# UltimateSoftware/surge

Measured on AMD Instinct MI355X. Metric: events/sec replayed, higher is better.
Workload: dtype int32/int64 adds + bit-copied f64

## Files before the change

### surge_amd/csrc/engine.hip

```cpp
#include <algorithm>
#include <atomic>
#include <cstdio>
#include <cstdlib>
#include <cstring>
#include <mutex>
#include <new>
#include <shared_mutex>
#include <string>
#include <vector>

#include "replay_internal.h"
#include "f64_text.h"
#include "state_parse.h"

using namespace surge;

namespace {

thread_local std::string g_last_error;

struct DevBuf {
  void* ptr = nullptr;
  size_t cap = 0;
  hipError_t reserve(size_t bytes) {
// ... 50 lines not shown
  std::mutex err_mu;

  DevBuf own_seg_off, own_events, own_init, own_state;
  const int64_t* d_seg_off = nullptr;
  const uint4* d_events = nullptr;
  const uint4* d_init = nullptr;
  uint4* d_state = nullptr;
  int64_t n_agg = 0, n_events = 0;
  bool bound = false;
  bool log_valid = false;

  CsrAnalysis an{};
  DevBuf d_analysis, nz_off, nz_map, block_counts;
  int64_t n_nz = 0;
  DevBuf perm, counter;
  DevBuf ix_arena, ix_cnt;
  bool perm_valid = false;
  struct ChunkIndex {
    DevBuf arena;
    void *v_start = nullptr, *v_len = nullptr, *v_info = nullptr, *v_seg = nullptr, *v_side = nullptr, *r_slot0 = nullptr, *r_c = nullptr, *r_out = nullptr;
    int64_t n_vrows = 0, n_cut_rows = 0;
    uint32_t T = 0;
    void release() {
      arena.release();
      v_start = v_len = v_info = v_seg = v_side = r_slot0 = r_c = r_out = nullptr;
      n_vrows = n_cut_rows = 0;
      T = 0;
    }
  };
  ChunkIndex cidx;
// ... 275 lines not shown
  if (extra) *extra = base + o_extra;
  return SURGE_OK;
}

void index_scratch_release(surge_replay_handle* h) {
  h->ix_arena.release();
  h->ix_cnt.release();
}

int32_t run_slots(surge_replay_handle* h, FoldParams& p, const int64_t* off, int64_t n_seg, bool cache_perm) {
  if (!cache_perm || !h->perm_valid) {
    HIPCHK(h, h->perm.reserve((size_t)(n_seg > 0 ? n_seg : 1) * 8));
    IndexScratch sc;
    const int32_t rcs = index_scratch(h, n_seg, false, cache_perm ? h->an.max_len : -1, 0, &sc);
    if (rcs != SURGE_OK) return rcs;
    HIPCHK(h, launch_sort_by_length(off, n_seg, sc, (int64_t*)h->perm.ptr, h->stream));
    h->perm_valid = cache_perm;
  }
  p.seg_off = off;
  p.plan = (const int64_t*)h->perm.ptr;
  {
    const int32_t rcd = dispenser_begin(h, p);
    if (rcd != SURGE_OK) return rcd;
  }
  p.n_seg = n_seg;
  const int64_t groups = (n_seg + kWave - 1) / kWave;
  const int le = env_lane_events("SURGE_REPLAY_LE_SLOTS", h->spec ? 16 : 8) == 16 ? 16 : 8;
  int64_t per_cu = le == 8 ? (h->spec ? 12 : 14) : 8;
  if (const char* v = std::getenv("SURGE_REPLAY_SLOTS_WAVES")) per_cu = std::atoi(v) > 0 ? std::atoi(v) : per_cu;
  const int64_t slots = (int64_t)h->n_cus * per_cu;
  const int64_t n_waves = groups < slots ? groups : slots;
  hipEvent_t e0, e1;
// ... 155 lines not shown
  if (!h) return SURGE_OK;
  DeviceGuard g(h->device);
  (void)hipStreamSynchronize(h->stream);
  if (h->comm) comm_destroy(h->comm);
  h->comm = nullptr;
  for (int k = 0; k < 2; ++k) {
    if (h->pinned[k]) (void)hipHostFree(h->pinned[k]);
    h->pinned[k] = nullptr;
    if (h->ev_staged[k]) (void)hipEventDestroy(h->ev_staged[k]);
    h->ev_staged[k] = nullptr;
  }
  if (h->host_flags) (void)hipHostFree(h->host_flags);
  h->host_flags = nullptr;
  h->cidx.release();
  h->tidx.release();
  DevBuf* bufs[] = {&h->gb_temp, &h->gb_u32, &h->gb_flags, &h->gb_agg_idx, &h->gb_events, &h->published, &h->gathered[0], &h->gathered[1], &h->f64_tables, &h->nan_count, &h->sd_ptab, &h->sd_counts, &h->sd_last, &h->sd_status, &h->ix_arena, &h->ix_cnt, &h->stage_keys, &h->stage_events, &h->t_tiles, &h->t_gsub, &h->perm, &h->counter, &h->own_seg_off, &h->own_events, &h->own_init, &h->own_state, &h->d_analysis, &h->nz_off,
                    &h->nz_map, &h->block_counts, &h->plan, &h->batch_group_agg, &h->batch_group_off,
                    &h->batch_events, &h->poison_count, &h->gather_idx, &h->gather_out, &h->scan_totals};
  for (DevBuf* b : bufs) b->release();
  hipEvent_t evs[] = {h->ev_total0, h->ev_total1, h->ev_h0, h->ev_h1, h->ev_i0, h->ev_i1, h->ev_r0, h->ev_r1};
  for (hipEvent_t ev : evs)
    if (ev) (void)hipEventDestroy(ev);
  for (auto& pr : h->fold_events) {
    (void)hipEventDestroy(pr.first);
    (void)hipEventDestroy(pr.second);
  }
  delete h;
  return SURGE_OK;
}

const char* surge_replay_last_error(const surge_replay_handle* h) {
// ... 29 lines not shown
}

int32_t surge_replay_bind_device_csr(surge_replay_handle* h, const int64_t* d_seg_off, int64_t n_agg,
                                     const void* d_events, int64_t n_events, const void* d_init_state,
                                     void* d_state_out) {
  if (!h) return fail(nullptr, SURGE_E_INVALID, "handle is NULL");
  if (n_agg < 0 || n_events < 0) return fail(h, SURGE_E_INVALID, "negative size");
  if (!d_seg_off) return fail(h, SURGE_E_INVALID, "seg_off is NULL");
  if (n_events > 0 && !d_events) return fail(h, SURGE_E_INVALID, "events is NULL");
  if (((uintptr_t)d_events & 15) || ((uintptr_t)d_init_state & 15) || ((uintptr_t)d_state_out & 15) ||
      ((uintptr_t)d_seg_off & 7))
    return fail(h, SURGE_E_INVALID, "device buffers must be 16-byte aligned (seg_off: 8)");
  DeviceGuard g(h->device);
  h->bound = false;
  h->perm_valid = false;
  h->cidx.T = 0;
  h->tidx.T = 0;
  h->tiled_valid = false;
  h->index_timed = h->relayout_timed = false;
  h->index_algo = 0;
  h->d_seg_off = d_seg_off;
  h->d_events = (const uint4*)d_events;
  h->d_init = (const uint4*)d_init_state;
  h->n_agg = n_agg;
  h->n_events = n_events;
  if (d_state_out) {
    h->d_state = (uint4*)d_state_out;
  } else {
    HIPCHK(h, h->own_state.reserve((size_t)n_agg * 64));
    h->d_state = (uint4*)h->own_state.ptr;
// ... 141 lines not shown
                               (int64_t*)ci.v_start, (uint32_t*)ci.v_len, (uint32_t*)ci.v_info, (int64_t*)ci.v_seg,
                               (int64_t*)ci.r_slot0, (uint32_t*)ci.r_c, (int64_t*)ci.r_out, h->stream));
  ci.T = T;
  return SURGE_OK;
}

int32_t ensure_index(surge_replay_handle* h, const FoldPlan& pl) {
  if (h->n_agg <= 0 || pl.span <= 0) return SURGE_OK;
  const int64_t* off = h->an.n_empty > 0 ? (const int64_t*)h->nz_off.ptr : h->d_seg_off;
  const int64_t n_seg = h->an.n_empty > 0 ? h->n_nz : h->n_agg;
  if (pl.use == SURGE_ALGO_SORTED && !h->perm_valid) {
    HIPCHK(h, h->perm.reserve((size_t)n_seg * 8));
    IndexScratch sc;
    const int32_t rcs = index_scratch(h, n_seg, false, h->an.max_len, 0, &sc);
    if (rcs != SURGE_OK) return rcs;
    HIPCHK(h, hipEventRecord(h->ev_i0, h->stream));
    HIPCHK(h, launch_sort_by_length(off, n_seg, sc, (int64_t*)h->perm.ptr, h->stream));
    HIPCHK(h, hipEventRecord(h->ev_i1, h->stream));
    h->perm_valid = true;
    h->index_timed = true;
    h->relayout_timed = false;
    h->index_algo = SURGE_ALGO_SORTED;
  } else if (pl.use == SURGE_ALGO_CHUNKED && h->cidx.T != pl.chunk_T) {
    HIPCHK(h, hipEventRecord(h->ev_i0, h->stream));
    const int32_t rc = build_chunk_index(h, h->cidx, off, n_seg, pl.chunk_T, true);
    if (rc != SURGE_OK) return rc;
    HIPCHK(h, hipEventRecord(h->ev_i1, h->stream));
    h->index_timed = true;
    h->relayout_timed = false;
    h->index_algo = SURGE_ALGO_CHUNKED;
  } else if (pl.use == SURGE_ALGO_TILED && (!h->tiled_valid || h->tidx.T != pl.chunk_T)) {
    h->tiled_valid = false;
    HIPCHK(h, hipEventRecord(h->ev_i0, h->stream));
    const int32_t rc = build_chunk_index(h, h->tidx, off, n_seg, pl.chunk_T, false);
// ... 275 lines not shown
      p.n_seg = h->n_agg;
      hipEvent_t e0, e1;
      const int32_t rc = next_fold_events(h, &e0, &e1);
      if (rc != SURGE_OK) return rc;
      HIPCHK(h, hipEventRecord(e0, h->stream));
      HIPCHK(h, launch_fold_short(p, h->stream));
      HIPCHK(h, hipEventRecord(e1, h->stream));
      h->st.n_tasks = (int32_t)((h->n_agg + 63) / 64);
    } else if (use == SURGE_ALGO_SORTED) {
      const int le = env_lane_events("SURGE_REPLAY_LE_SORTED", 16);
      const int64_t* off = h->an.n_empty > 0 ? (const int64_t*)h->nz_off.ptr : h->d_seg_off;
      const int64_t n_seg = h->an.n_empty > 0 ? h->n_nz : h->n_agg;
      if (h->an.n_empty > 0) p.out_map = (const int64_t*)h->nz_map.ptr;
      p.seg_off = off;
      p.plan = (const int64_t*)h->perm.ptr;
      {
        const int32_t rcd = dispenser_begin(h, p);
        if (rcd != SURGE_OK) return rcd;
      }
      p.n_seg = n_seg;
      const int64_t groups = (n_seg + kWave - 1) / kWave;
      int64_t per_cu = le == 8 ? 12 : (le == 16 ? 8 : 4);
      if (const char* v = std::getenv("SURGE_REPLAY_SORTED_WAVES")) per_cu = std::atoi(v) > 0 ? std::atoi(v) : per_cu;
      const int64_t slots = (int64_t)h->n_cus * per_cu;
      const int64_t n_waves = groups < slots ? groups : slots;
      hipEvent_t e0, e1;
      const int32_t rc = next_fold_events(h, &e0, &e1);
      if (rc != SURGE_OK) return rc;
      const V1Kernels* lanes = lane_spec(h, p);
      HIPCHK(h, hipEventRecord(e0, h->stream));
// ... 82 lines not shown
  if (n_groups == 0 || n_events == 0) return SURGE_OK;
  if (!d_group_agg || !d_group_off || !d_events) return fail(h, SURGE_E_INVALID, "NULL batch buffer");
  if ((uintptr_t)d_events & 15) return fail(h, SURGE_E_INVALID, "events must be 16-byte aligned");
  DeviceGuard g(h->device);
  FoldParams p;
  fill_params(h, p);
  p.events = (const uint4*)d_events;
  p.n_events = n_events;
  p.init = h->d_state;
  p.out = h->d_state;
  p.out_map = d_group_agg;
  HIPCHK(h, hipEventRecord(h->ev_total0, h->stream));
  if (h->v2) std::memset(p.table, 0, sizeof(p.table));
  const int32_t rc = h->v2 ? run_slots(h, p, d_group_off, n_groups, false) : run_flat(h, p, d_group_off, n_groups, n_events);
  if (rc != SURGE_OK) return rc;
  if (h->v2) h->perm_valid = false;
  HIPCHK(h, hipEventRecord(h->ev_total1, h->stream));
  h->timing_valid = true;
  h->st.last_algo = h->v2 ? SURGE_ALGO_SLOTS : SURGE_ALGO_FLAT;
  h->st.n_folds += 1;
  h->st.n_poisoned = -1;
  h->fold_epoch.fetch_add(1);
  return SURGE_OK;
}

int32_t surge_replay_append_fold(surge_replay_handle* h, const int64_t* group_agg, const int64_t* group_off,
                                 int64_t n_groups, const void* events, int64_t n_events) {
  if (!h) return fail(nullptr, SURGE_E_INVALID, "handle is NULL");
  if (!h->bound) return fail(h, SURGE_E_STATE, "append_fold before load_csr/bind_device_csr");
  if (n_groups < 0 || n_events < 0) return fail(h, SURGE_E_INVALID, "negative size");
  if (n_groups == 0 || n_events == 0) return SURGE_OK;
// ... 991 lines not shown
```

### surge_amd/csrc/fold_chunked.hip

```cpp
#include <cstdlib>
#include <cstring>

#include "fold_lane_device.h"

namespace surge {
namespace {

typedef const __attribute__((address_space(1))) void* gptr_t;
typedef __attribute__((address_space(3))) void* lptr_t;

__global__ void chunk_stitch_kernel(const FoldParams p, const uint32_t* __restrict__ side, const int64_t* __restrict__ r_slot0,
                                    const uint32_t* __restrict__ r_c, const int64_t* __restrict__ r_out, int64_t n_rows) {
  const int64_t r = (int64_t)blockIdx.x * blockDim.x + threadIdx.x;
  if (r >= n_rows) return;
  const int64_t slot0 = r_slot0[r];
  const uint32_t c = r_c[r];
  const int64_t oi = r_out[r];
  Acc x = p.init ? load_state(p.init, oi) : acc_none();
  for (uint32_t k = 0; k < c; ++k) {
    uint32_t w[kSideDwords];
    const uint4* q = (const uint4*)(side + (slot0 + k) * kSideDwords);
#pragma unroll
    for (int i = 0; i < 5; ++i) { const uint4 v = q[i]; w[4 * i] = v.x; w[4 * i + 1] = v.y; w[4 * i + 2] = v.z; w[4 * i + 3] = v.w; }
    const Acc P = acc_from_words(w);
// ... 4 lines not shown
  }
  store_state(p.out, oi, x);
}

template <int LE, bool CONC>
__global__ void __launch_bounds__(kWave) __attribute__((amdgpu_waves_per_eu(LE == 8 ? 3 : 2)))
fold_chunked_kernel(const FoldParams p, const ChunkTable t) {
  chunk_walk<LE, false, CONC>(p, t);
}

template <int LE, bool CONC>
__global__ void __launch_bounds__(kWave) __attribute__((amdgpu_waves_per_eu(LE == 8 ? 3 : 2)))
fold_sorted_pf_kernel(const FoldParams p) {
  ChunkTable t;
  t.v_start = nullptr; t.v_len = nullptr; t.v_info = nullptr; t.v_dest = nullptr; t.n_vrows = 0; t.side = nullptr;
  chunk_walk<LE, true, CONC>(p, t);
}

bool concrete_walk() {
  static const bool v = [] { const char* e = std::getenv("SURGE_REPLAY_WALK"); return !(e && std::strcmp(e, "transformer") == 0); }();
  return v;
}

}

hipError_t launch_fold_sorted_pf(const FoldParams& p, const V1Kernels* lanes, int64_t n_waves, int lane_events, hipStream_t stream) {
  if (n_waves <= 0) return hipSuccess;
  if (lanes) {
    const char* padv = std::getenv("SURGE_REPLAY_RTC_LDS_PAD");
    const unsigned pad = padv ? (unsigned)std::atoi(padv) : 0u;
    if (lane_events == 32) return launch_v1_lane(lanes->sorted32, &p, sizeof(p), n_waves, Geo<32>::kTileBytes + Geo<32>::kAuxSorted + pad, stream);
// ... 49 lines not shown
```

### surge_amd/csrc/fold_device.h

```cpp
#pragma once
#ifdef __HIPCC_RTC__
#include "fold_layout.h"
#else
#include "replay_internal.h"
#endif

namespace surge {
namespace {

typedef const __attribute__((address_space(1))) void* gptr_t;
typedef __attribute__((address_space(3))) void* lptr_t;

#ifndef SURGE_LOAD_AUX
#define SURGE_LOAD_AUX 2
#endif
constexpr int kLoadAux = SURGE_LOAD_AUX;

#ifdef SURGE_V1_SPEC
constexpr bool kSpecV1 = true;
#else
constexpr bool kSpecV1 = false;
#define SURGE_V1_MASK(k) 0u
#define SURGE_V1_THROWS 0u
#define SURGE_V1_DELETES 0u
// ... 206 lines not shown
  const uint32_t lo = __builtin_amdgcn_readfirstlane((uint32_t)v), hi = __builtin_amdgcn_readfirstlane((uint32_t)((uint64_t)v >> 32));
  return (int64_t)(((uint64_t)hi << 32) | lo);
}

__device__ __forceinline__ Acc readlane_acc(const Acc& a, int lane) {
  Acc r;
  r.count = (int32_t)rl((uint32_t)a.count, lane); r.version = (int32_t)rl((uint32_t)a.version, lane);
  r.sum = (int64_t)(((uint64_t)rl((uint32_t)((uint64_t)a.sum >> 32), lane) << 32) | rl((uint32_t)a.sum, lane));
  r.bal = ((uint64_t)rl((uint32_t)(a.bal >> 32), lane) << 32) | rl((uint32_t)a.bal, lane);
  r.mn = (int32_t)rl((uint32_t)a.mn, lane); r.mx = (int32_t)rl((uint32_t)a.mx, lane);
  r.n = rl(a.n, lane); r.fl = rl(a.fl, lane);
  return r;
}

__device__ __forceinline__ void store_state(uint4* out, int64_t idx, const Acc& a) {
  const bool pr = (a.fl & FL_PRESENT) != 0;
  uint4 v0, v1, v2, v3;
  v0.x = pr ? (uint32_t)a.count : 0u; v0.y = pr ? (uint32_t)a.version : 0u;
  v0.z = pr ? (uint32_t)a.sum : 0u; v0.w = pr ? (uint32_t)((uint64_t)a.sum >> 32) : 0u;
  v1.x = pr ? (uint32_t)a.bal : 0u; v1.y = pr ? (uint32_t)(a.bal >> 32) : 0u;
  v1.z = pr ? (uint32_t)a.mn : 0u; v1.w = pr ? (uint32_t)a.mx : 0u;
  v2.x = pr ? a.n : 0u; v2.y = a.fl & (FL_PRESENT | FL_POISONED); v2.z = 0u; v2.w = 0u;
  v3.x = v3.y = v3.z = v3.w = 0u;
  uint4* o = out + idx * 4;
  o[0] = v0; o[1] = v1; o[2] = v2; o[3] = v3;
}

__device__ __forceinline__ void store_state_flat(const FoldParams& p, int64_t idx, const Acc& a) {
  if (!kAnyDead) {
    store_state(p.out, idx, a);
// ... 217 lines not shown
```

### surge_amd/csrc/fold_kernels.hip

```cpp
#include <cstdio>
#include <cstdlib>
#include <cstring>
#include <map>
#include <memory>
#include <mutex>
#include <string>
#include <vector>

#include "fold_flat_device.h"
#include "fold_lane_device.h"

namespace surge {
namespace {

template <int MODE, int LE>
__global__ void __launch_bounds__(kWave) fold_kernel(const FoldParams p) {
  extern __shared__ __attribute__((aligned(16))) char smem[];
  fold_flat_body<MODE, LE>(p, smem);
}

template <int LE, bool CONC>
__global__ void __launch_bounds__(kWave) fold_rows_kernel(const FoldParams p) {
  __shared__ __attribute__((aligned(16))) char lds_ev[Geo<LE>::kTileBytes];
  __shared__ __attribute__((aligned(16))) uint32_t lds_tab[kTableLdsDwords];
// ... 385 lines not shown
  extern __shared__ __attribute__((aligned(16))) char smem[];
  fold_flat_body<MODE_FLAT, 8>(p, smem);
}
extern "C" __global__ void __launch_bounds__(64) surge_v1_flat16(const FoldParams p) {
  extern __shared__ __attribute__((aligned(16))) char smem[];
  fold_flat_body<MODE_FLAT, 16>(p, smem);
}
)SRC";
  } else {
    s += R"SRC(
#include "fold_lane_device.h"
using namespace surge;
extern "C" __global__ void __launch_bounds__(64) __attribute__((amdgpu_waves_per_eu(3))) surge_v1_sorted8(const FoldParams p) {
  ChunkTable t;
  t.v_start = nullptr; t.v_len = nullptr; t.v_info = nullptr; t.v_dest = nullptr; t.n_vrows = 0; t.side = nullptr;
  chunk_walk<8, true, true>(p, t);
}
extern "C" __global__ void __launch_bounds__(64) __attribute__((amdgpu_waves_per_eu(2))) surge_v1_sorted16(const FoldParams p) {
  ChunkTable t;
  t.v_start = nullptr; t.v_len = nullptr; t.v_info = nullptr; t.v_dest = nullptr; t.n_vrows = 0; t.side = nullptr;
  chunk_walk<16, true, true>(p, t);
}
extern "C" __global__ void __launch_bounds__(64) __attribute__((amdgpu_waves_per_eu(1))) surge_v1_sorted32(const FoldParams p) {
  ChunkTable t;
  t.v_start = nullptr; t.v_len = nullptr; t.v_info = nullptr; t.v_dest = nullptr; t.n_vrows = 0; t.side = nullptr;
  chunk_walk<32, true, true>(p, t);
}
extern "C" __global__ void __launch_bounds__(64) __attribute__((amdgpu_waves_per_eu(3))) surge_v1_chunked8(const ChunkArgs a) {
  chunk_walk<8, false, true>(a.p, a.t);
}
extern "C" __global__ void __launch_bounds__(64) __attribute__((amdgpu_waves_per_eu(2))) surge_v1_chunked16(const ChunkArgs a) {
  chunk_walk<16, false, true>(a.p, a.t);
}
extern "C" __global__ void __launch_bounds__(64) surge_v1_rows8(const FoldParams p) {
  __shared__ __attribute__((aligned(16))) char lds_ev[Geo<8>::kTileBytes];
  fold_rows_body<8, true>(p, lds_ev, nullptr);
}
extern "C" __global__ void __launch_bounds__(64) surge_v1_rows16(const FoldParams p) {
  __shared__ __attribute__((aligned(16))) char lds_ev[Geo<16>::kTileBytes];
  fold_rows_body<16, true>(p, lds_ev, nullptr);
}
// ... 157 lines not shown
```

### surge_amd/csrc/fold_lane_device.h

```cpp
#pragma once
#include "fold_chunk_device.h"

namespace surge {
namespace {

template <int V>
struct IntC { static constexpr int value = V; };

template <int LE, bool PERM, bool CONC>
__device__ __forceinline__ void chunk_walk(const FoldParams& p, const ChunkTable& t) {
  using G = Geo<LE>;
  extern __shared__ __attribute__((aligned(16))) char smem[];
  char* lds_ev = smem;
  int64_t* lds_rs = (int64_t*)(smem + G::kTileBytes);
  uint32_t* lds_len = (uint32_t*)(smem + G::kTileBytes + kWave * 8);
#ifdef SURGE_EXP_STATIC_TABLE
  __shared__ __attribute__((aligned(16))) uint32_t lds_tab_static[kTableLdsDwords];
  uint32_t* lds_tab = lds_tab_static;
#else
  uint32_t* lds_tab = (uint32_t*)(smem + G::kTileBytes + G::kAuxSorted);
#endif
  const int lane = threadIdx.x;
  load_table<LE>(p, lds_tab, lane);
  const uint32_t ev_row = G::ev_row(lane);
  const int64_t n_rows = PERM ? p.n_seg : t.n_vrows;
  const int64_t n_groups = (n_rows + kWave - 1) / kWave;

  auto grab = [&]() -> int64_t {
    unsigned long long g = 0;
    if (lane == 0) g = atomicAdd(p.counter, 1ull);
    return (int64_t)(((uint64_t)rl((uint32_t)(g >> 32), 0) << 32) | rl((uint32_t)g, 0));
  };
  struct Meta { int64_t dest, start; uint32_t len, info; };
  auto load_meta = [&](int64_t g) -> Meta {
    Meta m; m.dest = -1; m.start = 0; m.len = 0u; m.info = 0u;
    const int64_t idx = g * kWave + lane;
    if (g < n_groups && idx < n_rows) {
      if constexpr (PERM) {
        const int64_t sg = p.plan[idx];
        const int64_t st = p.seg_off[sg];
        const uint32_t pad = (uint32_t)(st & 7);
        m.dest = p.out_map ? p.out_map[sg] : sg;
        m.start = st - pad;
        m.len = (uint32_t)(p.seg_off[sg + 1] - st) + pad;
        m.info = pad << VI_PAD_SHIFT;
      } else {
        m.dest = t.v_dest[idx]; m.start = t.v_start[idx]; m.len = t.v_len[idx]; m.info = t.v_info[idx];
      }
    }
    return m;
  };
  struct Shape { uint32_t maxlen, minlen; int n_tiles; };
  auto shape_of = [&](const Meta& m) -> Shape {
    Shape sh;
    sh.maxlen = m.len;
    sh.minlen = m.len ? m.len : 0xffffffffu;
#pragma unroll
    for (int d = 32; d >= 1; d >>= 1) {
      sh.maxlen = max(sh.maxlen, (uint32_t)__shfl_xor((int)sh.maxlen, d, 64));
      sh.minlen = min(sh.minlen, (uint32_t)__shfl_xor((int)sh.minlen, d, 64));
    }
    sh.n_tiles = (int)((sh.maxlen + LE - 1) / LE);
    return sh;
  };
  auto publish = [&](const Meta& m) {
    lds_rs[lane] = m.start;
// ... 25 lines not shown
      asm volatile("" : "+v"(lane_o));
#pragma unroll
      for (int q = 0; q < G::kLoads; ++q) {
        const int r = G::kRowsPerLoad * q + lane_o / LE;
        const uint32_t rlen = lds_len[r];
        uint32_t j = (uint32_t)c * LE + G::load_j(lane_o, q % G::kClasses);
        const uint32_t lastj = rlen ? rlen - 1u : 0u;
        j = j < lastj ? j : lastj;
        __builtin_amdgcn_global_load_lds((gptr_t)(p.events + (lds_rs[r] + j)), (lptr_t)(lds_ev + q * 1024), 16, 0, kLoadAux);
      }
    }
  };

  int64_t g = grab();
  Meta cur = load_meta(g);
  Shape sh = shape_of(cur);
  publish(cur);
  if (g < n_groups) issue(0, sh.minlen);
  while (g < n_groups) {
    const int64_t g_next = grab();
    const Meta nxt = load_meta(g_next);
    Shape sh_next = sh;
    const uint32_t minlen = sh.minlen;
    const int n_tiles = sh.n_tiles;

    const uint32_t pad = (cur.info >> VI_PAD_SHIFT) & 7u;
    const bool whole = PERM || (cur.info & VI_RELATIVE) == 0u;
    Acc a = whole ? ((p.init && cur.dest >= 0) ? load_state(p.init, cur.dest) : acc_none()) : acc_identity();
    Acc P = acc_identity();
    uint32_t undecM = whole ? 0u : ~0u;
    uint32_t frozenM = whole ? (uint32_t)__builtin_amdgcn_sbfe((int32_t)a.fl, 1, 1) : 0u;
    uint32_t corr = 0u;
    const bool any_relative = !PERM && __builtin_amdgcn_ballot_w64(!whole) != 0ull;
    bool watching = any_relative;
    uint32_t presentM = (uint32_t)__builtin_amdgcn_sbfe((int32_t)a.fl, 0, 1);
    auto tile_step = [&](int c, auto tracking) {
      asm volatile("s_waitcnt vmcnt(0)" ::: "memory");
      uint4 ev[LE];
#pragma unroll
      for (int j = 0; j < LE; ++j) ev[j] = *(const uint4*)(lds_ev + (ev_row ^ (uint32_t)(j * 16)));
      asm volatile("s_waitcnt lgkmcnt(0)" ::: "memory");
      if (c + 1 < n_tiles) {
        issue(c + 1, minlen);
      } else {
        sh_next = shape_of(nxt);
        publish(nxt);
        if (g_next < n_groups) issue(0, sh_next.minlen);
      }

      uint32_t tyc[LE];
      if (c > 0 && (uint32_t)(c + 1) * LE <= minlen) {
#pragma unroll
        for (int j = 0; j < LE; ++j) tyc[j] = type_off(ev[j].x);
      } else {
        const int32_t rem = (int32_t)cur.len - c * LE;
        const int32_t skip = c == 0 ? (int32_t)pad : 0;
#pragma unroll
        for (int j = 0; j < LE; ++j)
          tyc[j] = (j >= skip && j < rem) ? type_off(ev[j].x) : kNullEntryOffBytes;
// ... 125 lines not shown
```

### surge_amd/csrc/fold_layout.h

```cpp
#pragma once

#ifdef __HIPCC_RTC__
typedef signed char int8_t;
typedef unsigned char uint8_t;
typedef short int16_t;
typedef unsigned short uint16_t;
typedef int int32_t;
typedef unsigned int uint32_t;
typedef long int64_t;
typedef unsigned long uint64_t;
#else
#include <stdint.h>

#include <hip/hip_runtime.h>
#endif

namespace surge {

constexpr int kWave = 64;
constexpr int kTaskBytes = 256 * 1024;
constexpr int kTableEntries = 18;
constexpr int kTableWords = 16;
constexpr int kTableStride = 20;
constexpr int kNullEntryOff = 17 * kTableStride + 24;
// ... 15 lines not shown
  TW_MIN = 12,
  TW_MAX = 13,
  TW_MATERIALIZES = 14,
  TW_FLAGS = 15,
};
constexpr int kTableWalkWords = 14;
constexpr int kTargetTasks = 8192;

struct FoldParams {
  const uint4* events;
  int64_t n_events;
  const int64_t* seg_off;
  const int64_t* plan;
  unsigned long long* counter;
  const int64_t* out_map;
  const uint4* init;
  uint4* out;
  int64_t n_seg;
  int64_t fixed_len;
  int64_t segs_per_task;
  uint32_t table[kTableEntries][kTableWords];
  int32_t d_count, d_version;
  int64_t d_sum;
  uint64_t d_balance;
  int32_t d_min, d_max;
  uint32_t d_evcount;
};

struct TileTable {
  const uint4* tiles;
// ... 12 lines not shown
```

### surge_amd/csrc/index_kernels.hip

```cpp
#include "fold_chunk_device.h"

namespace surge {
namespace {

constexpr uint32_t kLenKeyMax = 65535u;

__global__ void length_keys_kernel(const int64_t* __restrict__ off, int64_t n_seg, uint32_t* __restrict__ keys, int64_t* __restrict__ vals) {
  const int64_t s = (int64_t)blockIdx.x * blockDim.x + threadIdx.x;
  if (s >= n_seg) return;
  const int64_t len = off[s + 1] - off[s];
  keys[s] = len < (int64_t)kLenKeyMax ? (uint32_t)len : kLenKeyMax;
  vals[s] = s;
}

__host__ __device__ __forceinline__ uint32_t chunks_of(int64_t span, uint32_t T) {
  const int64_t c = (span + T - 1) / T;
  return (uint32_t)(c < 1 ? 1 : c);
}

__global__ void chunk_count_kernel(const int64_t* __restrict__ off, int64_t n_seg, uint32_t T, bool align, int64_t* __restrict__ cnt,
                                   int64_t stride) {
  const int64_t s = (int64_t)blockIdx.x * blockDim.x + threadIdx.x;
  if (s >= n_seg) return;
  const int64_t st = off[s], len = off[s + 1] - st;
// ... 35 lines not shown
    keys[pos] = vl < kLenKeyMax ? vl : kLenKeyMax;
    if (vals) vals[pos] = pos;
  }
}

__global__ void chunk_gather_kernel(const int64_t* __restrict__ order, int64_t n, const int64_t* __restrict__ u_start,
                                    const uint32_t* __restrict__ u_len, const uint32_t* __restrict__ u_info, const int64_t* __restrict__ u_dest,
                                    int64_t* __restrict__ v_start, uint32_t* __restrict__ v_len, uint32_t* __restrict__ v_info,
                                    int64_t* __restrict__ v_dest) {
  const int64_t i = (int64_t)blockIdx.x * blockDim.x + threadIdx.x;
  if (i >= n) return;
  const int64_t src = order[i];
  v_start[i] = u_start[src]; v_len[i] = u_len[src]; v_info[i] = u_info[src]; v_dest[i] = u_dest[src];
}

}

hipError_t launch_sort_by_length(const int64_t* off, int64_t n_seg, const IndexScratch& sc, int64_t* perm, hipStream_t stream) {
  if (n_seg <= 0) return hipSuccess;
  if (sc.counting) return launch_count_sort_desc(nullptr, off, n_seg, sc.max_key, sc.n_cus, sc.temp, perm, stream);
  hipLaunchKernelGGL(length_keys_kernel, dim3((unsigned)((n_seg + 255) / 256)), dim3(256), 0, stream, off, n_seg, sc.keys_a, sc.vals_a);
  return launch_radix_sort_pairs_desc(sc.temp, sc.temp_bytes, sc.keys_a, sc.keys_b, sc.vals_a, perm, n_seg, stream);
}

hipError_t launch_chunk_count(const int64_t* off, int64_t n_seg, uint32_t T, bool align, int64_t* cnt, void* scan_scratch, hipStream_t stream) {
  if (n_seg <= 0) return hipSuccess;
  const int64_t stride = n_seg + 1;
  hipLaunchKernelGGL(chunk_count_kernel, dim3((unsigned)((n_seg + 255) / 256)), dim3(256), 0, stream, off, n_seg, T, align, cnt, stride);
  for (int k = 0; k < 3; ++k) {
    hipError_t e = hipMemsetAsync(cnt + k * stride + n_seg, 0, 8, stream);
    if (e != hipSuccess) return e;
  }
  return launch_exclusive_scans_i64(cnt, stride, stride, 3, scan_scratch, stream);
}

hipError_t launch_chunk_table(const int64_t* off, int64_t n_seg, const int64_t* out_map, uint32_t T, bool align, const int64_t* cnt,
                              int64_t n_vrows, const IndexScratch& sc, int64_t* u_start, uint32_t* u_len, uint32_t* u_info, int64_t* u_dest,
                              int64_t* v_start, uint32_t* v_len, uint32_t* v_info, int64_t* v_dest, int64_t* r_slot0, uint32_t* r_c,
                              int64_t* r_out, hipStream_t stream) {
  if (n_seg <= 0 || n_vrows <= 0) return hipSuccess;
  hipLaunchKernelGGL(chunk_emit_kernel, dim3((unsigned)((n_seg + 255) / 256)), dim3(256), 0, stream, off, n_seg, out_map, T, align, cnt,
                     n_seg + 1, u_start, u_len, u_info, u_dest, sc.keys_a, sc.vals_a, r_slot0, r_c, r_out);
  hipError_t e;
  if (sc.counting) {
    e = launch_count_sort_desc(sc.keys_a, nullptr, n_vrows, sc.max_key, sc.n_cus, sc.temp, sc.vals_b, stream);
  } else {
    e = launch_radix_sort_pairs_desc(sc.temp, sc.temp_bytes, sc.keys_a, sc.keys_b, sc.vals_a, sc.vals_b, n_vrows, stream);
  }
  if (e != hipSuccess) return e;
  hipLaunchKernelGGL(chunk_gather_kernel, dim3((unsigned)((n_vrows + 255) / 256)), dim3(256), 0, stream, sc.vals_b, n_vrows, u_start, u_len,
                     u_info, u_dest, v_start, v_len, v_info, v_dest);
  return hipGetLastError();
}

}
```

### surge_amd/csrc/length_sort.hip

```cpp
#include "replay_internal.h"

namespace surge {
namespace {

constexpr int kLsRowsPerSlab = 64;

__device__ __forceinline__ uint32_t ls_key(const uint32_t* __restrict__ keys, const int64_t* __restrict__ off, int64_t i) {
  if (keys) return keys[i];
  const int64_t len = off[i + 1] - off[i];
  return len < 65535 ? (uint32_t)len : 65535u;
}

__device__ __forceinline__ unsigned long long ls_peers(uint32_t key, bool valid, int bits) {
  unsigned long long peers = __ballot(valid);
  for (int b = 0; b < bits; ++b) {
    const bool bit = ((key >> b) & 1u) != 0u;
    const unsigned long long m = __ballot(bit);
    peers &= bit ? m : ~m;
  }
  return peers;
}

__global__ void __launch_bounds__(64) ls_hist_kernel(const uint32_t* __restrict__ keys, const int64_t* __restrict__ off, int64_t n, int64_t per,
                                                     int bins, int bits, uint32_t* __restrict__ hm) {
// ... 72 lines not shown

__global__ void ls_cursor_kernel(uint32_t* __restrict__ hm, int n_rows, int bins, const uint32_t* __restrict__ part, const uint32_t* __restrict__ base) {
  const int bin = blockIdx.x * blockDim.x + threadIdx.x;
  const int slab = blockIdx.y;
  if (bin >= bins) return;
  const int r0 = slab * kLsRowsPerSlab;
  const int r1 = r0 + kLsRowsPerSlab < n_rows ? r0 + kLsRowsPerSlab : n_rows;
  uint32_t run = base[bin] + part[(size_t)slab * bins + bin];
  for (int r = r0; r < r1; ++r) {
    const uint32_t v = hm[(size_t)r * bins + bin];
    hm[(size_t)r * bins + bin] = run;
    run += v;
  }
}

__global__ void __launch_bounds__(64) ls_scatter_kernel(const uint32_t* __restrict__ keys, const int64_t* __restrict__ off, int64_t n, int64_t per,
                                                        int bins, int bits, const uint32_t* __restrict__ hm, int64_t* __restrict__ perm) {
  extern __shared__ uint32_t ls_lds[];
  const int lane = threadIdx.x;
  const uint32_t* row = hm + (size_t)blockIdx.x * bins;
  for (int b = lane; b < bins; b += 64) ls_lds[b] = row[b];
  const int64_t s0 = (int64_t)blockIdx.x * per;
  int64_t s1 = s0 + per;
  s1 = s1 < n ? s1 : n;
  const unsigned long long below = lane == 0 ? 0ull : (~0ull >> (64 - lane));
  int64_t i = s0 + lane;
  uint32_t key_next = i < s1 ? ls_key(keys, off, i) : 0u;
  for (int64_t base = s0; base < s1; base += 64) {
    const bool valid = i < s1;
    const uint32_t key = key_next;
    const int64_t me = i;
    i += 64;
    key_next = i < s1 ? ls_key(keys, off, i) : 0u;
    const unsigned long long peers = ls_peers(key, valid, bits);
    const uint32_t c0 = valid ? ls_lds[key] : 0u;
    const bool leader = valid && (__ffsll((long long)peers) - 1 == lane);
    if (leader) ls_lds[key] = c0 + (uint32_t)__popcll(peers);
    if (valid) perm[(int64_t)c0 + __popcll(peers & below)] = me;
  }
}

constexpr int kScanBlock = 256, kScanItems = 8, kScanTile = kScanBlock * kScanItems;

__device__ __forceinline__ int64_t block_exclusive_scan(int64_t v, int64_t* s_wave, int64_t* total) {
  const int lane = threadIdx.x & 63, wave = threadIdx.x >> 6;
  int64_t inc = v;
#pragma unroll
  for (int d = 1; d < 64; d <<= 1) {
    const int64_t o = __shfl_up(inc, d, 64);
    if (lane >= d) inc += o;
  }
  if (lane == 63) s_wave[wave] = inc;
  __syncthreads();
// ... 65 lines not shown
  p = (p + 63) / 64 * 64;
  if (p < 256) p = 256;
  *per = p;
  *n_waves = (n + p - 1) / p;
}

size_t count_sort_scratch_bytes(int64_t n, uint32_t max_key, int n_cus) {
  int64_t per, waves;
  count_sort_shape(n > 0 ? n : 1, n_cus, &per, &waves);
  const size_t bins = (size_t)max_key + 1;
  const size_t slabs = (size_t)((waves + kLsRowsPerSlab - 1) / kLsRowsPerSlab);
  return ((size_t)waves * bins + slabs * bins + bins) * 4 + 256;
}

hipError_t launch_count_sort_desc(const uint32_t* keys, const int64_t* off, int64_t n, uint32_t max_key, int n_cus, void* scratch, int64_t* perm,
                                  hipStream_t stream) {
  if (n <= 0) return hipSuccess;
  if (max_key >= (uint32_t)kCountSortMaxBins) return hipErrorInvalidValue;
  int64_t per, waves;
  count_sort_shape(n, n_cus, &per, &waves);
  const int bins = (int)max_key + 1;
  int bits = 0;
  while ((1u << bits) < (uint32_t)bins) ++bits;
  const int slabs = (int)((waves + kLsRowsPerSlab - 1) / kLsRowsPerSlab);
  uint32_t* hm = (uint32_t*)scratch;
  uint32_t* part = hm + (size_t)waves * bins;
  uint32_t* total = part + (size_t)slabs * bins;
  const unsigned lds = (unsigned)bins * 4u;
  hipLaunchKernelGGL(ls_hist_kernel, dim3((unsigned)waves), dim3(64), lds, stream, keys, off, n, per, bins, bits, hm);
  const dim3 g2((unsigned)((bins + 255) / 256), (unsigned)slabs);
  hipLaunchKernelGGL(ls_slab_sum_kernel, g2, dim3(256), 0, stream, (const uint32_t*)hm, (int)waves, bins, part);
  hipLaunchKernelGGL(ls_slab_scan_kernel, dim3((unsigned)((bins + 255) / 256)), dim3(256), 0, stream, part, slabs, bins, total);
  hipLaunchKernelGGL(ls_bin_scan_kernel, dim3(1), dim3(1024), 0, stream, total, bins);
  hipLaunchKernelGGL(ls_cursor_kernel, g2, dim3(256), 0, stream, hm, (int)waves, bins, (const uint32_t*)part, (const uint32_t*)total);
  hipLaunchKernelGGL(ls_scatter_kernel, dim3((unsigned)waves), dim3(64), lds, stream, keys, off, n, per, bins, bits, (const uint32_t*)hm, perm);
  return hipGetLastError();
}

size_t scan_i64_scratch_bytes(int64_t n, int k_arrays) {
  const int64_t nb = (n + kScanTile - 1) / kScanTile;
  return (size_t)k_arrays * (size_t)(nb + 1) * 8;
}

hipError_t launch_exclusive_scans_i64(int64_t* v, int64_t n, int64_t stride, int k_arrays, void* scratch, hipStream_t stream) {
  if (n <= 0 || k_arrays <= 0) return hipSuccess;
  const int64_t nb = (n + kScanTile - 1) / kScanTile;
  int64_t* sums = (int64_t*)scratch;
  hipLaunchKernelGGL(scan_reduce_kernel, dim3((unsigned)nb, (unsigned)k_arrays), dim3(kScanBlock), 0, stream, (const int64_t*)v, n, stride, sums, nb);
  hipLaunchKernelGGL(scan_sums_kernel, dim3((unsigned)k_arrays), dim3(kScanBlock), 0, stream, sums, nb);
  hipLaunchKernelGGL(scan_apply_kernel, dim3((unsigned)nb, (unsigned)k_arrays), dim3(kScanBlock), 0, stream, v, n, stride, (const int64_t*)sums, nb);
// ... 5 lines not shown
```

### surge_amd/csrc/replay_internal.h

```cpp
#pragma once

#include <hip/hip_runtime.h>
#include <stdint.h>

#include <string>
#include <vector>

#include "../../include/surge_replay.h"
#include "fold_layout.h"

namespace surge {

struct CsrAnalysis {
  int32_t bad;
  int32_t nonuniform;
  int64_t n_empty;
  int64_t len0;
  int64_t max_len;
  int64_t first, last;
};

hipError_t launch_fold_fixed(const FoldParams& p, int64_t n_tasks, int lane_events, hipStream_t stream);
enum { V1_FLAT = 0, V1_LANES = 1 };
struct V1Kernels {
// ... 14 lines not shown
struct IndexScratch {
  void* temp;
  size_t temp_bytes;
  uint32_t *keys_a, *keys_b;
  int64_t *vals_a, *vals_b;
  bool counting;
  uint32_t max_key;
  int n_cus;
};
hipError_t index_temp_bytes(int64_t n, size_t* bytes);
hipError_t launch_radix_sort_pairs_desc(void* temp, size_t temp_bytes, const uint32_t* keys_in, uint32_t* keys_out, const int64_t* vals_in,
                                        int64_t* vals_out, int64_t n, hipStream_t stream);
constexpr int kCountSortMaxBins = 8192;
size_t count_sort_scratch_bytes(int64_t n, uint32_t max_key, int n_cus);
hipError_t launch_count_sort_desc(const uint32_t* keys, const int64_t* off, int64_t n, uint32_t max_key, int n_cus, void* scratch, int64_t* perm,
                                  hipStream_t stream);
size_t scan_i64_scratch_bytes(int64_t n, int k_arrays);
hipError_t launch_exclusive_scans_i64(int64_t* v, int64_t n, int64_t stride, int k_arrays, void* scratch, hipStream_t stream);
hipError_t launch_sort_by_length(const int64_t* off, int64_t n_seg, const IndexScratch& sc, int64_t* perm, hipStream_t stream);
hipError_t launch_chunk_count(const int64_t* off, int64_t n_seg, uint32_t T, bool align, int64_t* cnt, void* scan_scratch, hipStream_t stream);
hipError_t launch_chunk_table(const int64_t* off, int64_t n_seg, const int64_t* out_map, uint32_t T, bool align, const int64_t* cnt,
                              int64_t n_vrows, const IndexScratch& sc, int64_t* u_start, uint32_t* u_len, uint32_t* u_info, int64_t* u_dest,
                              int64_t* v_start, uint32_t* v_len, uint32_t* v_info, int64_t* v_dest, int64_t* r_slot0, uint32_t* r_c,
                              int64_t* r_out, hipStream_t stream);
hipError_t launch_fold_chunked(const FoldParams& p, const int64_t* v_start, const uint32_t* v_len, const uint32_t* v_info,
                               const int64_t* v_dest, int64_t n_vrows, uint32_t* side, const int64_t* r_slot0, const uint32_t* r_c,
                               const int64_t* r_out, int64_t n_cut, const V1Kernels* lanes, int64_t n_waves, int lane_events, hipStream_t stream);
hipError_t launch_chunk_stitch(const FoldParams& p, const uint32_t* side, const int64_t* r_slot0, const uint32_t* r_c, const int64_t* r_out,
                               int64_t n_cut, hipStream_t stream);
constexpr int kTileSubBytes = 8192;
hipError_t launch_tile_index(const uint32_t* v_len, int64_t n_vrows, int64_t* g_sub, hipStream_t stream);
hipError_t launch_relayout(const uint4* events, const int64_t* v_start, const uint32_t* v_len, int64_t n_vrows, const int64_t* g_sub0,
                           int64_t n_sub_total, uint4* tiles, hipStream_t stream);
hipError_t launch_fold_tiled(const FoldParams& p, const uint4* tiles, const int64_t* g_sub0, const uint32_t* v_len,
// ... 95 lines not shown
```

Before: 373.4 billion.

## Precompute sorted row table to replace dependent plan/offset/map gathers in sorted fold

During the SORTED index build, a 16-byte row record (start, length, destination) is now written per sorted position. This happens either in the count-sort scatter or in a gather kernel after the radix sort. The sorted fold kernels then load one coalesced uint4 per lane instead of chasing perm -> seg_off -> out_map through several dependent random loads. The aim is to cut the latency of per-group metadata loads in the hot fold loop, at the cost of extra index-build work and an n_seg*16-byte buffer. It also adds an experiments-only macro that skips state stores.

```diff
diff --git a/surge_amd/csrc/engine.hip b/surge_amd/csrc/engine.hip
--- a/surge_amd/csrc/engine.hip
+++ b/surge_amd/csrc/engine.hip
@@ -88,6 +88,8 @@
   DevBuf d_analysis, nz_off, nz_map, block_counts;
   int64_t n_nz = 0;
   DevBuf perm, counter;
+  DevBuf rows;
+  bool rows_valid = false;
   DevBuf ix_arena, ix_cnt;
   bool perm_valid = false;
   struct ChunkIndex {
@@ -393,8 +395,9 @@
     IndexScratch sc;
     const int32_t rcs = index_scratch(h, n_seg, false, cache_perm ? h->an.max_len : -1, 0, &sc);
     if (rcs != SURGE_OK) return rcs;
-    HIPCHK(h, launch_sort_by_length(off, n_seg, sc, (int64_t*)h->perm.ptr, h->stream));
+    HIPCHK(h, launch_sort_by_length(off, n_seg, sc, (int64_t*)h->perm.ptr, nullptr, nullptr, h->stream));
     h->perm_valid = cache_perm;
+    h->rows_valid = false;
   }
   p.seg_off = off;
   p.plan = (const int64_t*)h->perm.ptr;
@@ -580,7 +583,7 @@
   h->host_flags = nullptr;
   h->cidx.release();
   h->tidx.release();
-  DevBuf* bufs[] = {&h->gb_temp, &h->gb_u32, &h->gb_flags, &h->gb_agg_idx, &h->gb_events, &h->published, &h->gathered[0], &h->gathered[1], &h->f64_tables, &h->nan_count, &h->sd_ptab, &h->sd_counts, &h->sd_last, &h->sd_status, &h->ix_arena, &h->ix_cnt, &h->stage_keys, &h->stage_events, &h->t_tiles, &h->t_gsub, &h->perm, &h->counter, &h->own_seg_off, &h->own_events, &h->own_init, &h->own_state, &h->d_analysis, &h->nz_off,
+  DevBuf* bufs[] = {&h->gb_temp, &h->gb_u32, &h->gb_flags, &h->gb_agg_idx, &h->gb_events, &h->published, &h->gathered[0], &h->gathered[1], &h->f64_tables, &h->nan_count, &h->sd_ptab, &h->sd_counts, &h->sd_last, &h->sd_status, &h->ix_arena, &h->ix_cnt, &h->stage_keys, &h->stage_events, &h->t_tiles, &h->t_gsub, &h->perm, &h->rows, &h->counter, &h->own_seg_off, &h->own_events, &h->own_init, &h->own_state, &h->d_analysis, &h->nz_off,
                     &h->nz_map, &h->block_counts, &h->plan, &h->batch_group_agg, &h->batch_group_off,
                     &h->batch_events, &h->poison_count, &h->gather_idx, &h->gather_out, &h->scan_totals};
   for (DevBuf* b : bufs) b->release();
@@ -640,6 +643,7 @@
   DeviceGuard g(h->device);
   h->bound = false;
   h->perm_valid = false;
+  h->rows_valid = false;
   h->cidx.T = 0;
   h->tidx.T = 0;
   h->tiled_valid = false;
@@ -811,10 +815,14 @@
     IndexScratch sc;
     const int32_t rcs = index_scratch(h, n_seg, false, h->an.max_len, 0, &sc);
     if (rcs != SURGE_OK) return rcs;
+    const bool table = n_seg < (1ll << 32) && h->n_agg <= (1ll << 32) && h->an.max_len < (1ll << 32) - 8;
+    if (table) HIPCHK(h, h->rows.reserve((size_t)n_seg * 16));
     HIPCHK(h, hipEventRecord(h->ev_i0, h->stream));
-    HIPCHK(h, launch_sort_by_length(off, n_seg, sc, (int64_t*)h->perm.ptr, h->stream));
+    HIPCHK(h, launch_sort_by_length(off, n_seg, sc, (int64_t*)h->perm.ptr, h->an.n_empty > 0 ? (const int64_t*)h->nz_map.ptr : nullptr,
+                                    table ? (uint4*)h->rows.ptr : nullptr, h->stream));
     HIPCHK(h, hipEventRecord(h->ev_i1, h->stream));
     h->perm_valid = true;
+    h->rows_valid = table;
     h->index_timed = true;
     h->relayout_timed = false;
     h->index_algo = SURGE_ALGO_SORTED;
@@ -1120,6 +1128,7 @@
       if (h->an.n_empty > 0) p.out_map = (const int64_t*)h->nz_map.ptr;
       p.seg_off = off;
       p.plan = (const int64_t*)h->perm.ptr;
+      p.rows = h->rows_valid ? (const uint4*)h->rows.ptr : nullptr;
       {
         const int32_t rcd = dispenser_begin(h, p);
         if (rcd != SURGE_OK) return rcd;
@@ -1232,7 +1241,7 @@
   if (h->v2) std::memset(p.table, 0, sizeof(p.table));
   const int32_t rc = h->v2 ? run_slots(h, p, d_group_off, n_groups, false) : run_flat(h, p, d_group_off, n_groups, n_events);
   if (rc != SURGE_OK) return rc;
-  if (h->v2) h->perm_valid = false;
+  if (h->v2) h->perm_valid = h->rows_valid = false;
   HIPCHK(h, hipEventRecord(h->ev_total1, h->stream));
   h->timing_valid = true;
   h->st.last_algo = h->v2 ? SURGE_ALGO_SLOTS : SURGE_ALGO_FLAT;
diff --git a/surge_amd/csrc/fold_chunked.hip b/surge_amd/csrc/fold_chunked.hip
--- a/surge_amd/csrc/fold_chunked.hip
+++ b/surge_amd/csrc/fold_chunked.hip
@@ -42,7 +42,8 @@
 fold_sorted_pf_kernel(const FoldParams p) {
   ChunkTable t;
   t.v_start = nullptr; t.v_len = nullptr; t.v_info = nullptr; t.v_dest = nullptr; t.n_vrows = 0; t.side = nullptr;
-  chunk_walk<LE, true, CONC>(p, t);
+  if (p.rows) chunk_walk<LE, true, CONC, true>(p, t);
+  else chunk_walk<LE, true, CONC, false>(p, t);
 }
 
 bool concrete_walk() {
diff --git a/surge_amd/csrc/fold_device.h b/surge_amd/csrc/fold_device.h
--- a/surge_amd/csrc/fold_device.h
+++ b/surge_amd/csrc/fold_device.h
@@ -244,6 +244,9 @@
 }
 
 __device__ __forceinline__ void store_state(uint4* out, int64_t idx, const Acc& a) {
+#if defined(SURGE_EXPERIMENTS) && defined(SURGE_EXP_NO_STATE_STORE)
+  if (((uint64_t)out & 15u) != 1u) return;
+#endif
   const bool pr = (a.fl & FL_PRESENT) != 0;
   uint4 v0, v1, v2, v3;
   v0.x = pr ? (uint32_t)a.count : 0u; v0.y = pr ? (uint32_t)a.version : 0u;
diff --git a/surge_amd/csrc/fold_kernels.hip b/surge_amd/csrc/fold_kernels.hip
--- a/surge_amd/csrc/fold_kernels.hip
+++ b/surge_amd/csrc/fold_kernels.hip
@@ -423,17 +423,20 @@
 extern "C" __global__ void __launch_bounds__(64) __attribute__((amdgpu_waves_per_eu(3))) surge_v1_sorted8(const FoldParams p) {
   ChunkTable t;
   t.v_start = nullptr; t.v_len = nullptr; t.v_info = nullptr; t.v_dest = nullptr; t.n_vrows = 0; t.side = nullptr;
-  chunk_walk<8, true, true>(p, t);
+  if (p.rows) chunk_walk<8, true, true, true>(p, t);
+  else chunk_walk<8, true, true, false>(p, t);
 }
 extern "C" __global__ void __launch_bounds__(64) __attribute__((amdgpu_waves_per_eu(2))) surge_v1_sorted16(const FoldParams p) {
   ChunkTable t;
   t.v_start = nullptr; t.v_len = nullptr; t.v_info = nullptr; t.v_dest = nullptr; t.n_vrows = 0; t.side = nullptr;
-  chunk_walk<16, true, true>(p, t);
+  if (p.rows) chunk_walk<16, true, true, true>(p, t);
+  else chunk_walk<16, true, true, false>(p, t);
 }
 extern "C" __global__ void __launch_bounds__(64) __attribute__((amdgpu_waves_per_eu(1))) surge_v1_sorted32(const FoldParams p) {
   ChunkTable t;
   t.v_start = nullptr; t.v_len = nullptr; t.v_info = nullptr; t.v_dest = nullptr; t.n_vrows = 0; t.side = nullptr;
-  chunk_walk<32, true, true>(p, t);
+  if (p.rows) chunk_walk<32, true, true, true>(p, t);
+  else chunk_walk<32, true, true, false>(p, t);
 }
 extern "C" __global__ void __launch_bounds__(64) __attribute__((amdgpu_waves_per_eu(3))) surge_v1_chunked8(const ChunkArgs a) {
   chunk_walk<8, false, true>(a.p, a.t);
diff --git a/surge_amd/csrc/fold_lane_device.h b/surge_amd/csrc/fold_lane_device.h
--- a/surge_amd/csrc/fold_lane_device.h
+++ b/surge_amd/csrc/fold_lane_device.h
@@ -7,8 +7,9 @@
 template <int V>
 struct IntC { static constexpr int value = V; };
 
-template <int LE, bool PERM, bool CONC>
+template <int LE, bool PERM, bool CONC, bool TABLE = false>
 __device__ __forceinline__ void chunk_walk(const FoldParams& p, const ChunkTable& t) {
+  static_assert(PERM || !TABLE, "the row table is SORTED's");
   using G = Geo<LE>;
   extern __shared__ __attribute__((aligned(16))) char smem[];
   char* lds_ev = smem;
@@ -35,6 +36,15 @@
   auto load_meta = [&](int64_t g) -> Meta {
     Meta m; m.dest = -1; m.start = 0; m.len = 0u; m.info = 0u;
     const int64_t idx = g * kWave + lane;
+    if constexpr (PERM && TABLE) {
+      const bool mine = g < n_groups && idx < n_rows;
+      const uint4 e = p.rows[mine ? idx : 0];
+      m.dest = (int64_t)(uint64_t)e.w;
+      m.start = (int64_t)(((uint64_t)e.y << 32) | e.x);
+      m.len = e.z;
+      m.info = mine ? 0u : 1u;
+      return m;
+    }
     if (g < n_groups && idx < n_rows) {
       if constexpr (PERM) {
         const int64_t sg = p.plan[idx];
@@ -50,6 +60,16 @@
     }
     return m;
   };
+  auto finish_meta = [&](Meta& m) {
+    if constexpr (TABLE) {
+      const bool mine = m.info == 0u;
+      const uint32_t pad = mine ? (uint32_t)m.start & 7u : 0u;
+      m.dest = mine ? m.dest : -1;
+      m.start = mine ? m.start - pad : 0;
+      m.len = mine ? m.len + pad : 0u;
+      m.info = pad << VI_PAD_SHIFT;
+    }
+  };
   struct Shape { uint32_t maxlen, minlen; int n_tiles; };
   auto shape_of = [&](const Meta& m) -> Shape {
     Shape sh;
@@ -105,12 +125,13 @@
 
   int64_t g = grab();
   Meta cur = load_meta(g);
+  finish_meta(cur);
   Shape sh = shape_of(cur);
   publish(cur);
   if (g < n_groups) issue(0, sh.minlen);
   while (g < n_groups) {
     const int64_t g_next = grab();
-    const Meta nxt = load_meta(g_next);
+    Meta nxt = load_meta(g_next);
     Shape sh_next = sh;
     const uint32_t minlen = sh.minlen;
     const int n_tiles = sh.n_tiles;
@@ -134,6 +155,7 @@
       if (c + 1 < n_tiles) {
         issue(c + 1, minlen);
       } else {
+        finish_meta(nxt);
         sh_next = shape_of(nxt);
         publish(nxt);
         if (g_next < n_groups) issue(0, sh_next.minlen);
diff --git a/surge_amd/csrc/fold_layout.h b/surge_amd/csrc/fold_layout.h
--- a/surge_amd/csrc/fold_layout.h
+++ b/surge_amd/csrc/fold_layout.h
@@ -53,6 +53,7 @@
   const int64_t* plan;
   unsigned long long* counter;
   const int64_t* out_map;
+  const uint4* rows;
   const uint4* init;
   uint4* out;
   int64_t n_seg;
diff --git a/surge_amd/csrc/index_kernels.hip b/surge_amd/csrc/index_kernels.hip
--- a/surge_amd/csrc/index_kernels.hip
+++ b/surge_amd/csrc/index_kernels.hip
@@ -73,13 +73,27 @@
   v_start[i] = u_start[src]; v_len[i] = u_len[src]; v_info[i] = u_info[src]; v_dest[i] = u_dest[src];
 }
 
+__global__ void row_table_gather_kernel(const int64_t* __restrict__ perm, int64_t n, const int64_t* __restrict__ off, const int64_t* __restrict__ out_map,
+                                        uint4* __restrict__ rows) {
+  const int64_t r = (int64_t)blockIdx.x * blockDim.x + threadIdx.x;
+  if (r >= n) return;
+  const int64_t s = perm[r];
+  const int64_t st = off[s], len = off[s + 1] - st;
+  const int64_t dest = out_map ? out_map[s] : s;
+  rows[r] = make_uint4((uint32_t)st, (uint32_t)((uint64_t)st >> 32), (uint32_t)len, (uint32_t)dest);
 }
 
-hipError_t launch_sort_by_length(const int64_t* off, int64_t n_seg, const IndexScratch& sc, int64_t* perm, hipStream_t stream) {
+}
+
+hipError_t launch_sort_by_length(const int64_t* off, int64_t n_seg, const IndexScratch& sc, int64_t* perm, const int64_t* out_map, uint4* rows,
+                                 hipStream_t stream) {
   if (n_seg <= 0) return hipSuccess;
-  if (sc.counting) return launch_count_sort_desc(nullptr, off, n_seg, sc.max_key, sc.n_cus, sc.temp, perm, stream);
+  if (sc.counting) return launch_count_sort_desc(nullptr, off, n_seg, sc.max_key, sc.n_cus, sc.temp, perm, out_map, rows, stream);
   hipLaunchKernelGGL(length_keys_kernel, dim3((unsigned)((n_seg + 255) / 256)), dim3(256), 0, stream, off, n_seg, sc.keys_a, sc.vals_a);
-  return launch_radix_sort_pairs_desc(sc.temp, sc.temp_bytes, sc.keys_a, sc.keys_b, sc.vals_a, perm, n_seg, stream);
+  const hipError_t e = launch_radix_sort_pairs_desc(sc.temp, sc.temp_bytes, sc.keys_a, sc.keys_b, sc.vals_a, perm, n_seg, stream);
+  if (e != hipSuccess || !rows) return e;
+  hipLaunchKernelGGL(row_table_gather_kernel, dim3((unsigned)((n_seg + 255) / 256)), dim3(256), 0, stream, (const int64_t*)perm, n_seg, off, out_map, rows);
+  return hipGetLastError();
 }
 
 hipError_t launch_chunk_count(const int64_t* off, int64_t n_seg, uint32_t T, bool align, int64_t* cnt, void* scan_scratch, hipStream_t stream) {
@@ -102,7 +116,7 @@
                      n_seg + 1, u_start, u_len, u_info, u_dest, sc.keys_a, sc.vals_a, r_slot0, r_c, r_out);
   hipError_t e;
   if (sc.counting) {
-    e = launch_count_sort_desc(sc.keys_a, nullptr, n_vrows, sc.max_key, sc.n_cus, sc.temp, sc.vals_b, stream);
+    e = launch_count_sort_desc(sc.keys_a, nullptr, n_vrows, sc.max_key, sc.n_cus, sc.temp, sc.vals_b, nullptr, nullptr, stream);
   } else {
     e = launch_radix_sort_pairs_desc(sc.temp, sc.temp_bytes, sc.keys_a, sc.keys_b, sc.vals_a, sc.vals_b, n_vrows, stream);
   }
diff --git a/surge_amd/csrc/length_sort.hip b/surge_amd/csrc/length_sort.hip
--- a/surge_amd/csrc/length_sort.hip
+++ b/surge_amd/csrc/length_sort.hip
@@ -110,8 +110,10 @@
   }
 }
 
+template <bool ROWS>
 __global__ void __launch_bounds__(64) ls_scatter_kernel(const uint32_t* __restrict__ keys, const int64_t* __restrict__ off, int64_t n, int64_t per,
-                                                        int bins, int bits, const uint32_t* __restrict__ hm, int64_t* __restrict__ perm) {
+                                                        int bins, int bits, const uint32_t* __restrict__ hm, int64_t* __restrict__ perm,
+                                                        const int64_t* __restrict__ out_map, uint4* __restrict__ rows) {
   extern __shared__ uint32_t ls_lds[];
   const int lane = threadIdx.x;
   const uint32_t* row = hm + (size_t)blockIdx.x * bins;
@@ -121,18 +123,34 @@
   s1 = s1 < n ? s1 : n;
   const unsigned long long below = lane == 0 ? 0ull : (~0ull >> (64 - lane));
   int64_t i = s0 + lane;
-  uint32_t key_next = i < s1 ? ls_key(keys, off, i) : 0u;
+  int64_t st_next = 0, len_next = 0, dest_next = 0;
+  auto fetch = [&](int64_t r) -> uint32_t {
+    if constexpr (!ROWS) {
+      return r < s1 ? ls_key(keys, off, r) : 0u;
+    } else {
+      if (r >= s1) return 0u;
+      st_next = off[r];
+      len_next = off[r + 1] - st_next;
+      dest_next = out_map ? out_map[r] : r;
+      return len_next < 65535 ? (uint32_t)len_next : 65535u;
+    }
+  };
+  uint32_t key_next = fetch(i);
   for (int64_t base = s0; base < s1; base += 64) {
     const bool valid = i < s1;
     const uint32_t key = key_next;
-    const int64_t me = i;
+    const int64_t me = i, st = st_next, len = len_next, dest = dest_next;
     i += 64;
-    key_next = i < s1 ? ls_key(keys, off, i) : 0u;
+    key_next = fetch(i);
     const unsigned long long peers = ls_peers(key, valid, bits);
     const uint32_t c0 = valid ? ls_lds[key] : 0u;
     const bool leader = valid && (__ffsll((long long)peers) - 1 == lane);
     if (leader) ls_lds[key] = c0 + (uint32_t)__popcll(peers);
-    if (valid) perm[(int64_t)c0 + __popcll(peers & below)] = me;
+    if (valid) {
+      const int64_t pos = (int64_t)c0 + __popcll(peers & below);
+      perm[pos] = me;
+      if (ROWS) rows[pos] = make_uint4((uint32_t)st, (uint32_t)((uint64_t)st >> 32), (uint32_t)len, (uint32_t)dest);
+    }
   }
 }
 
@@ -228,9 +246,9 @@
 }
 
 hipError_t launch_count_sort_desc(const uint32_t* keys, const int64_t* off, int64_t n, uint32_t max_key, int n_cus, void* scratch, int64_t* perm,
-                                  hipStream_t stream) {
+                                  const int64_t* out_map, uint4* rows, hipStream_t stream) {
   if (n <= 0) return hipSuccess;
-  if (max_key >= (uint32_t)kCountSortMaxBins) return hipErrorInvalidValue;
+  if (max_key >= (uint32_t)kCountSortMaxBins || (rows && keys)) return hipErrorInvalidValue;
   int64_t per, waves;
   count_sort_shape(n, n_cus, &per, &waves);
   const int bins = (int)max_key + 1;
@@ -247,7 +265,8 @@
   hipLaunchKernelGGL(ls_slab_scan_kernel, dim3((unsigned)((bins + 255) / 256)), dim3(256), 0, stream, part, slabs, bins, total);
   hipLaunchKernelGGL(ls_bin_scan_kernel, dim3(1), dim3(1024), 0, stream, total, bins);
   hipLaunchKernelGGL(ls_cursor_kernel, g2, dim3(256), 0, stream, hm, (int)waves, bins, (const uint32_t*)part, (const uint32_t*)total);
-  hipLaunchKernelGGL(ls_scatter_kernel, dim3((unsigned)waves), dim3(64), lds, stream, keys, off, n, per, bins, bits, (const uint32_t*)hm, perm);
+  if (rows) hipLaunchKernelGGL(ls_scatter_kernel<true>, dim3((unsigned)waves), dim3(64), lds, stream, keys, off, n, per, bins, bits, (const uint32_t*)hm, perm, out_map, rows);
+  else hipLaunchKernelGGL(ls_scatter_kernel<false>, dim3((unsigned)waves), dim3(64), lds, stream, keys, off, n, per, bins, bits, (const uint32_t*)hm, perm, out_map, rows);
   return hipGetLastError();
 }
 
diff --git a/surge_amd/csrc/replay_internal.h b/surge_amd/csrc/replay_internal.h
--- a/surge_amd/csrc/replay_internal.h
+++ b/surge_amd/csrc/replay_internal.h
@@ -52,10 +52,11 @@
 constexpr int kCountSortMaxBins = 8192;
 size_t count_sort_scratch_bytes(int64_t n, uint32_t max_key, int n_cus);
 hipError_t launch_count_sort_desc(const uint32_t* keys, const int64_t* off, int64_t n, uint32_t max_key, int n_cus, void* scratch, int64_t* perm,
-                                  hipStream_t stream);
+                                  const int64_t* out_map, uint4* rows, hipStream_t stream);
 size_t scan_i64_scratch_bytes(int64_t n, int k_arrays);
 hipError_t launch_exclusive_scans_i64(int64_t* v, int64_t n, int64_t stride, int k_arrays, void* scratch, hipStream_t stream);
-hipError_t launch_sort_by_length(const int64_t* off, int64_t n_seg, const IndexScratch& sc, int64_t* perm, hipStream_t stream);
+hipError_t launch_sort_by_length(const int64_t* off, int64_t n_seg, const IndexScratch& sc, int64_t* perm, const int64_t* out_map, uint4* rows,
+                                 hipStream_t stream);
 hipError_t launch_chunk_count(const int64_t* off, int64_t n_seg, uint32_t T, bool align, int64_t* cnt, void* scan_scratch, hipStream_t stream);
 hipError_t launch_chunk_table(const int64_t* off, int64_t n_seg, const int64_t* out_map, uint32_t T, bool align, const int64_t* cnt,
                               int64_t n_vrows, const IndexScratch& sc, int64_t* u_start, uint32_t* u_len, uint32_t* u_info, int64_t* u_dest,
```

Result: no change. 376.2 billion, median of 2 (+0.7%).
